# basilevh/occlusions-4d

Hardware: AMD Instinct MI355X
Metric: 4D query-points/sec (encode+decode) at n_points=14336 (higher is better)
Workload: dtype f32; 1 GPU; GREATER inference (BASELINE configs[1]): n_points=14336 video_len=12 num_sample=524288 (-> 534528 grid queries) implicit_batch_size=32768 (decoded in mini-batches of 32256 = 3584 workgroups of 9 queries; every query is decoded, results do not depend on the split), seeded random-init weights; abstract_points=531, outputs_per_query=5, parallelism=single GPU, schedule=sequential, rccl_ranks=1, decode_streams=2, decode_chunk=32256

## Files before the change

occlusions-4d_amd/csrc/pointops.hip:

```cpp
#include "common.hpp"

namespace {

constexpr int TPB = 256;

inline dim3 grid1d(int64_t total) { return dim3((unsigned)((total + TPB - 1) / TPB)); }

__global__ __launch_bounds__(TPB) void pos_hidden_kernel(const float* __restrict__ pos, int64_t ps,
                                                         const float* __restrict__ pos2, int64_t p2s,
                                                         const int32_t* __restrict__ idx, int64_t total, int k, int h,
                                                         const float* __restrict__ P1, const float* __restrict__ c1,
                                                         float* __restrict__ out) {
  const int64_t e = (int64_t)blockIdx.x * TPB + threadIdx.x;
  if (e >= total) return;
  const int m = (int)(e % h);
  const int64_t p = e / h;
  const int64_t i = p / k;
  const int j = idx[p];
  const float* a = pos + i * ps;
  const float* b = pos2 + (int64_t)j * p2s;
  const float dx = a[0] - b[0], dy = a[1] - b[1], dz = a[2] - b[2];
  const float* w = P1 + 3 * m;
  float v = fmaf(dz, w[2], fmaf(dy, w[1], dx * w[0])) + c1[m];
  out[e] = fmaxf(v, 0.f);
}

__global__ __launch_bounds__(TPB) void attn_in_kernel(const float* __restrict__ q, int64_t ldq,
                                                      const float* __restrict__ kf, int64_t ldk,
                                                      const float* __restrict__ pe, const int32_t* __restrict__ idx,
                                                      int64_t total, int k, int d, float* __restrict__ out) {
  const int64_t e = (int64_t)blockIdx.x * TPB + threadIdx.x;
  if (e >= total) return;
  const int c = (int)(e % d);
  const int64_t p = e / d;
  const int64_t i = p / k;
  const int j = idx[p];
  out[e] = (q[i * ldq + c] - kf[(int64_t)j * ldk + c]) + pe[e];
}

template <int KMAX>
__global__ __launch_bounds__(TPB) void softmax_agg_kernel(const float* __restrict__ logits,
                                                          const float* __restrict__ v, int64_t ldv,
                                                          const float* __restrict__ pe,
                                                          const int32_t* __restrict__ idx, int64_t total, int k, int d,
                                                          float divisor, float* __restrict__ agg, int64_t ld_agg) {
  const int64_t e = (int64_t)blockIdx.x * TPB + threadIdx.x;
  if (e >= total) return;
  const int c = (int)(e % d);
  const int64_t i = e / d;
  float a[KMAX];
  float mx = -__builtin_inff();
#pragma unroll
  for (int j = 0; j < KMAX; ++j) {
    if (j < k) {
      a[j] = logits[(i * k + j) * d + c] / divisor;
      mx = fmaxf(mx, a[j]);
    }
  }
  float den = 0.f;
#pragma unroll
  for (int j = 0; j < KMAX; ++j) {
    if (j < k) {
      a[j] = expf(a[j] - mx);
      den += a[j];
    }
  }
  float s = 0.f;
#pragma unroll
  for (int j = 0; j < KMAX; ++j) {
    if (j < k) {
      const int64_t p = i * k + j;
      float val = v[(int64_t)idx[p] * ldv + c];
      if (pe) val += pe[p * d + c];
      s += (a[j] / den) * val;
    }
  }
  agg[i * ld_agg + c] = s;
}

__global__ __launch_bounds__(TPB) void layernorm_kernel(const float* __restrict__ x, int64_t ldx,
                                                        const float* __restrict__ gamma,
                                                        const float* __restrict__ beta, float eps, int relu_out,
                                                        float* __restrict__ y, int64_t ldy, int n, int d) {
  const int row = blockIdx.x * (TPB / 64) + (threadIdx.x >> 6);
  const int lane = threadIdx.x & 63;
  if (row >= n) return;
  const float* xr = x + (int64_t)row * ldx;
  float s = 0.f;
  for (int c = lane; c < d; c += 64) s += xr[c];
#pragma unroll
  for (int o = 32; o > 0; o >>= 1) s += __shfl_xor(s, o);
  const float mean = s / (float)d;
  float q = 0.f;
  for (int c = lane; c < d; c += 64) {
    const float t = xr[c] - mean;
    q += t * t;
  }
#pragma unroll
  for (int o = 32; o > 0; o >>= 1) q += __shfl_xor(q, o);
  const float rstd = 1.0f / sqrtf(q / (float)d + eps);
  float* yr = y + (int64_t)row * ldy;
  for (int c = lane; c < d; c += 64) {
    float t = (xr[c] - mean) * rstd;
    if (gamma) t = t * gamma[c] + beta[c];
    yr[c] = relu_out ? fmaxf(t, 0.f) : t;
  }
}

__global__ __launch_bounds__(TPB) void maxpool_gather_kernel(const float* __restrict__ y, int64_t ldy,
                                                             const int32_t* __restrict__ idx, int64_t total, int k,
                                                             int d, float* __restrict__ z, int64_t ldz) {
  const int64_t e = (int64_t)blockIdx.x * TPB + threadIdx.x;
  if (e >= total) return;
  const int c = (int)(e % d);
  const int64_t i = e / d;
  float m = y[(int64_t)idx[i * k] * ldy + c];
  for (int j = 1; j < k; ++j) m = fmaxf(m, y[(int64_t)idx[i * k + j] * ldy + c]);
  z[i * ldz + c] = m;
}

__global__ __launch_bounds__(TPB) void gather_rows_kernel(const float* __restrict__ src, int64_t lds,
                                                          const int32_t* __restrict__ idx, int64_t total, int d,
                                                          float* __restrict__ out, int64_t ldo) {
  const int64_t e = (int64_t)blockIdx.x * TPB + threadIdx.x;
  if (e >= total) return;
  const int c = (int)(e % d);
  const int64_t i = e / d;
  out[i * ldo + c] = src[(int64_t)idx[i] * lds + c];
}

__global__ __launch_bounds__(TPB) void mean_rows_kernel(const float* __restrict__ x, int64_t ldx, int n, int d,
                                                        float* __restrict__ out) {
  static_assert(TPB == 256, "mean_rows_kernel assumes 256 threads");
  __shared__ float part[8][32];
  const int cl = threadIdx.x & 31, g = threadIdx.x >> 5;
  const int c = blockIdx.x * 32 + cl;
  float s = 0.f;
  if (c < d)
    for (int i = g; i < n; i += 8) s += x[(int64_t)i * ldx + c];
  part[g][cl] = s;
  __syncthreads();
  if (g == 0 && c < d) {
    float t = part[0][cl];
#pragma unroll
    for (int k = 1; k < 8; ++k) t += part[k][cl];
    out[c] = t / (float)n;
  }
}

struct PosencFreqs { float w[16]; };

__global__ __launch_bounds__(TPB) void posenc_kernel(const float* __restrict__ pts, int64_t stride, int64_t total,
                                                     int c, int width, PosencFreqs fr, float* __restrict__ out,
                                                     int64_t ldo) {
  const int64_t e = (int64_t)blockIdx.x * TPB + threadIdx.x;
  if (e >= total) return;
  const int col = (int)(e % width);
  const int64_t i = e / width;
  const float* p = pts + i * stride;
  float v;
  if (col < c) {
    v = p[col];
  } else {
    const int f = (col - c) / (2 * c), r = (col - c) % (2 * c);
    const float arg = p[r % c] * fr.w[f];
    v = r < c ? sinf(arg) : cosf(arg);
  }
  out[i * ldo + col] = v;
}

__global__ __launch_bounds__(TPB) void interp_weights_kernel(const float* __restrict__ dist, int n, int k,
                                                             float* __restrict__ w) {
  const int i = blockIdx.x * TPB + threadIdx.x;
  if (i >= n) return;
  float s = 0.f;
  for (int j = 0; j < k; ++j) {
    const float t = 1.0f / (dist[(int64_t)i * k + j] + 1e-4f);
    w[(int64_t)i * k + j] = t;
    s += fabsf(t);
  }
  s = fmaxf(s, 1e-12f);
  for (int j = 0; j < k; ++j) w[(int64_t)i * k + j] = w[(int64_t)i * k + j] / s;
}

__global__ __launch_bounds__(TPB) void interp_add_kernel(float* __restrict__ x, int64_t ldx,
                                                         const float* __restrict__ cvec,
                                                         const float* __restrict__ table, int64_t ldt,
                                                         const int32_t* __restrict__ idx, const float* __restrict__ w,
                                                         int64_t total, int k, int d) {
  const int64_t e = (int64_t)blockIdx.x * TPB + threadIdx.x;
  if (e >= total) return;
  const int c = (int)(e % d);
  const int64_t i = e / d;
  float s = 0.f;
  for (int j = 0; j < k; ++j) s += w[i * k + j] * table[(int64_t)idx[i * k + j] * ldt + c];
  if (cvec) s += cvec[c];
  x[i * ldx + c] += s;
}

template <int KC>
__global__ __launch_bounds__(TPB) void interp_add4_kernel(float* __restrict__ x, int64_t ldx,
                                                          const float* __restrict__ cvec,
                                                          const float* __restrict__ table, int64_t ldt,
                                                          const int32_t* __restrict__ idx, const float* __restrict__ w,
                                                          int64_t total, int k, int d4) {
  typedef float f4 __attribute__((ext_vector_type(4)));
  const int64_t e = (int64_t)blockIdx.x * TPB + threadIdx.x;
  if (e >= total) return;
  const int c = 4 * (int)(e % d4);
  const int64_t i = e / d4;
  f4 s = {0.f, 0.f, 0.f, 0.f};
  if (KC > 0) {
    int jj[KC > 0 ? KC : 1];
    float wj[KC > 0 ? KC : 1];
    f4 t[KC > 0 ? KC : 1];
#pragma unroll
    for (int j = 0; j < KC; ++j) { jj[j] = idx[i * KC + j]; wj[j] = w[i * KC + j]; }
#pragma unroll
    for (int j = 0; j < KC; ++j) t[j] = *reinterpret_cast<const f4*>(table + (int64_t)jj[j] * ldt + c);
#pragma unroll
    for (int j = 0; j < KC; ++j) { s.x += wj[j] * t[j].x; s.y += wj[j] * t[j].y; s.z += wj[j] * t[j].z; s.w += wj[j] * t[j].w; }
  } else {
    for (int j = 0; j < k; ++j) {
      const float wj = w[i * k + j];
      const f4 t = *reinterpret_cast<const f4*>(table + (int64_t)idx[i * k + j] * ldt + c);
      s.x += wj * t.x; s.y += wj * t.y; s.z += wj * t.z; s.w += wj * t.w;
    }
  }
  if (cvec) {
    const f4 cv = *reinterpret_cast<const f4*>(cvec + c);
    s.x += cv.x; s.y += cv.y; s.z += cv.z; s.w += cv.w;
  }
  f4* xp = reinterpret_cast<f4*>(x + i * ldx + c);
  f4 xv = *xp;
  xv.x += s.x; xv.y += s.y; xv.z += s.z; xv.w += s.w;
  *xp = xv;
}

struct SquashOps { int32_t op[32]; };

__global__ __launch_bounds__(TPB) void squash_kernel(float* __restrict__ out, int64_t ld, int64_t total, int g,
                                                     SquashOps ops) {
  const int64_t e = (int64_t)blockIdx.x * TPB + threadIdx.x;
  if (e >= total) return;
  const int c = (int)(e % g);
  const int64_t i = e / g;
  float v = out[i * ld + c];
  const int op = ops.op[c];
  if (op == 1) v = 1.0f / (1.0f + expf(-v));
  else if (op == 2) v = fminf(fmaxf(v, 0.f), 1.f);
  out[i * ld + c] = v;
}


__global__ __launch_bounds__(256) void matmul_f64_kernel(const double* __restrict__ A, int64_t sam, int64_t sak,
                                                         const double* __restrict__ B, int64_t sbk, int64_t sbn,
                                                         double* __restrict__ Cm, int M, int N, int K) {
  __shared__ double sa[16][17], sb[16][17];
  const int tx = threadIdx.x & 15, ty = threadIdx.x >> 4;
  const int m = blockIdx.y * 16 + ty, n = blockIdx.x * 16 + tx;
  double acc = 0.0;
  for (int k0 = 0; k0 < K; k0 += 16) {
    const int ka = k0 + tx, kb = k0 + ty;
    sa[ty][tx] = (m < M && ka < K) ? A[(int64_t)m * sam + (int64_t)ka * sak] : 0.0;
    sb[ty][tx] = (kb < K && n < N) ? B[(int64_t)kb * sbk + (int64_t)n * sbn] : 0.0;
    __syncthreads();
#pragma unroll
    for (int kk = 0; kk < 16; ++kk) acc = fma(sa[ty][kk], sb[kk][tx], acc);
    __syncthreads();
  }
  if (m < M && n < N) Cm[(int64_t)m * N + n] = acc;
}

}

extern "C" {

int occ4d_pt_pos_hidden_f32(const float* pos, int64_t ps, const float* pos2, int64_t p2s, const int32_t* idx,
                            int n, int k, const float* P1, const float* c1, int h, float* out, void* stream) {
  OCC4D_REQUIRE(pos && pos2 && idx && P1 && c1 && out, "occ4d_pt_pos_hidden_f32: null pointer");
  OCC4D_REQUIRE(n >= 0 && k >= 1 && h >= 1 && ps >= 3 && p2s >= 3, "occ4d_pt_pos_hidden_f32: bad sizes");
  const int64_t total = (int64_t)n * k * h;
  if (!total) return OCC4D_OK;
  pos_hidden_kernel<<<grid1d(total), TPB, 0, (hipStream_t)stream>>>(pos, ps, pos2, p2s, idx, total, k, h, P1, c1, out);
  return occ4d::check_launch("occ4d_pt_pos_hidden_f32");
}

int occ4d_pt_attn_in_f32(const float* q, int64_t ldq, const float* kfeat, int64_t ldk, const float* pe,
                         const int32_t* idx, int n, int k, int d, float* out, void* stream) {
  OCC4D_REQUIRE(q && kfeat && pe && idx && out, "occ4d_pt_attn_in_f32: null pointer");
  OCC4D_REQUIRE(n >= 0 && k >= 1 && d >= 1 && ldq >= d && ldk >= d, "occ4d_pt_attn_in_f32: bad sizes");
  const int64_t total = (int64_t)n * k * d;
  if (!total) return OCC4D_OK;
  attn_in_kernel<<<grid1d(total), TPB, 0, (hipStream_t)stream>>>(q, ldq, kfeat, ldk, pe, idx, total, k, d, out);
  return occ4d::check_launch("occ4d_pt_attn_in_f32");
}

int occ4d_pt_softmax_agg_f32(const float* logits, const float* v, int64_t ldv, const float* pe, const int32_t* idx,
                             int n, int k, int d, float divisor, float* agg, int64_t ld_agg, void* stream) {
  OCC4D_REQUIRE(logits && v && idx && agg, "occ4d_pt_softmax_agg_f32: null pointer");
  OCC4D_REQUIRE(n >= 0 && k >= 1 && k <= 16 && d >= 1 && ldv >= d && ld_agg >= d, "occ4d_pt_softmax_agg_f32: bad sizes");
  OCC4D_REQUIRE(divisor > 0.f, "occ4d_pt_softmax_agg_f32: divisor must be > 0");
  const int64_t total = (int64_t)n * d;
  if (!total) return OCC4D_OK;
  softmax_agg_kernel<16><<<grid1d(total), TPB, 0, (hipStream_t)stream>>>(logits, v, ldv, pe, idx, total, k, d, divisor, agg, ld_agg);
  return occ4d::check_launch("occ4d_pt_softmax_agg_f32");
}

int occ4d_layernorm_f32(const float* x, int64_t ldx, const float* gamma, const float* beta, float eps, int relu_out,
                        float* y, int64_t ldy, int n, int d, void* stream) {
  OCC4D_REQUIRE(x && y, "occ4d_layernorm_f32: null pointer");
  OCC4D_REQUIRE((gamma == nullptr) == (beta == nullptr), "occ4d_layernorm_f32: gamma/beta must both be set or NULL");
  OCC4D_REQUIRE(n >= 0 && d >= 1 && ldx >= d && ldy >= d, "occ4d_layernorm_f32: bad sizes");
  if (!n) return OCC4D_OK;
  layernorm_kernel<<<occ4d::cdiv(n, TPB / 64), TPB, 0, (hipStream_t)stream>>>(x, ldx, gamma, beta, eps, relu_out, y, ldy, n, d);
  return occ4d::check_launch("occ4d_layernorm_f32");
}

int occ4d_maxpool_gather_f32(const float* y, int64_t ldy, const int32_t* idx, int n_out, int k, int d, float* z,
                             int64_t ldz, void* stream) {
  OCC4D_REQUIRE(y && idx && z, "occ4d_maxpool_gather_f32: null pointer");
  OCC4D_REQUIRE(n_out >= 0 && k >= 1 && d >= 1 && ldy >= d && ldz >= d, "occ4d_maxpool_gather_f32: bad sizes");
  const int64_t total = (int64_t)n_out * d;
  if (!total) return OCC4D_OK;
  maxpool_gather_kernel<<<grid1d(total), TPB, 0, (hipStream_t)stream>>>(y, ldy, idx, total, k, d, z, ldz);
  return occ4d::check_launch("occ4d_maxpool_gather_f32");
}

int occ4d_gather_rows_f32(const float* src, int64_t lds, const int32_t* idx, int n_out, int d, float* out,
                          int64_t ldo, void* stream) {
  OCC4D_REQUIRE(src && idx && out, "occ4d_gather_rows_f32: null pointer");
  OCC4D_REQUIRE(n_out >= 0 && d >= 1 && lds >= d && ldo >= d, "occ4d_gather_rows_f32: bad sizes");
  const int64_t total = (int64_t)n_out * d;
  if (!total) return OCC4D_OK;
  gather_rows_kernel<<<grid1d(total), TPB, 0, (hipStream_t)stream>>>(src, lds, idx, total, d, out, ldo);
  return occ4d::check_launch("occ4d_gather_rows_f32");
}

int occ4d_mean_rows_f32(const float* x, int64_t ldx, int n, int d, float* out, void* stream) {
  OCC4D_REQUIRE(x && out, "occ4d_mean_rows_f32: null pointer");
  OCC4D_REQUIRE(n >= 1 && d >= 1 && ldx >= d, "occ4d_mean_rows_f32: bad sizes");
  mean_rows_kernel<<<occ4d::cdiv(d, 32), TPB, 0, (hipStream_t)stream>>>(x, ldx, n, d, out);
  return occ4d::check_launch("occ4d_mean_rows_f32");
}

int occ4d_posenc_f32(const float* pts, int64_t stride, int n, int c, int n_freq, double base_freq, float* out,
                     int64_t ldo, void* stream) {
  OCC4D_REQUIRE(pts && out, "occ4d_posenc_f32: null pointer");
  OCC4D_REQUIRE(n >= 0 && c >= 1 && n_freq >= 0 && n_freq <= 16 && stride >= c, "occ4d_posenc_f32: bad sizes");
  const int width = c * (2 * n_freq + 1);
  OCC4D_REQUIRE(ldo >= width, "occ4d_posenc_f32: ldo too small");
  PosencFreqs fr;
  for (int f = 0; f < 16; ++f) {
    const double omega = base_freq * (double)(1u << f) * 3.141592653589793 * 2.0;
    fr.w[f] = (float)omega;
  }
  const int64_t total = (int64_t)n * width;
  if (!total) return OCC4D_OK;
  posenc_kernel<<<grid1d(total), TPB, 0, (hipStream_t)stream>>>(pts, stride, total, c, width, fr, out, ldo);
  return occ4d::check_launch("occ4d_posenc_f32");
}

int occ4d_interp_weights_f32(const float* dist, int n, int k, float* w, void* stream) {
  OCC4D_REQUIRE(dist && w, "occ4d_interp_weights_f32: null pointer");
  OCC4D_REQUIRE(n >= 0 && k >= 1, "occ4d_interp_weights_f32: bad sizes");
  if (!n) return OCC4D_OK;
  interp_weights_kernel<<<occ4d::cdiv(n, TPB), TPB, 0, (hipStream_t)stream>>>(dist, n, k, w);
  return occ4d::check_launch("occ4d_interp_weights_f32");
}

int occ4d_interp_add_f32(float* x, int64_t ldx, const float* cvec, const float* table, int64_t ldt,
                         const int32_t* idx, const float* w, int n, int k, int d, void* stream) {
  OCC4D_REQUIRE(x && table && idx && w, "occ4d_interp_add_f32: null pointer");
  OCC4D_REQUIRE(n >= 0 && k >= 1 && d >= 1 && ldx >= d && ldt >= d, "occ4d_interp_add_f32: bad sizes");
  const int64_t total = (int64_t)n * d;
  if (!total) return OCC4D_OK;
  const bool vec = d % 4 == 0 && ldx % 4 == 0 && ldt % 4 == 0 && ((uintptr_t)x % 16) == 0 &&
                   ((uintptr_t)table % 16) == 0 && (!cvec || ((uintptr_t)cvec % 16) == 0);
  if (vec) {
    const int64_t total4 = (int64_t)n * (d / 4);
    if (k == 8)
      interp_add4_kernel<8><<<grid1d(total4), TPB, 0, (hipStream_t)stream>>>(x, ldx, cvec, table, ldt, idx, w, total4, k, d / 4);
    else
      interp_add4_kernel<0><<<grid1d(total4), TPB, 0, (hipStream_t)stream>>>(x, ldx, cvec, table, ldt, idx, w, total4, k, d / 4);
  } else {
    interp_add_kernel<<<grid1d(total), TPB, 0, (hipStream_t)stream>>>(x, ldx, cvec, table, ldt, idx, w, total, k, d);
  }
  return occ4d::check_launch("occ4d_interp_add_f32");
}

int occ4d_squash_f32(float* out, int64_t ld, int n, int g, const int32_t* ops_host, void* stream) {
  OCC4D_REQUIRE(out && ops_host, "occ4d_squash_f32: null pointer");
  OCC4D_REQUIRE(n >= 0 && g >= 1 && g <= 32 && ld >= g, "occ4d_squash_f32: need 1 <= g <= 32, ld >= g");
  SquashOps ops;
  for (int i = 0; i < 32; ++i) ops.op[i] = i < g ? ops_host[i] : 0;
  for (int i = 0; i < g; ++i) OCC4D_REQUIRE(ops.op[i] >= 0 && ops.op[i] <= 2, "occ4d_squash_f32: op code %d", ops.op[i]);
  const int64_t total = (int64_t)n * g;
  if (!total) return OCC4D_OK;
  squash_kernel<<<grid1d(total), TPB, 0, (hipStream_t)stream>>>(out, ld, total, g, ops);
  return occ4d::check_launch("occ4d_squash_f32");
}

}

extern "C" int occ4d_matmul_f64(const double* a, int64_t sam, int64_t sak, const double* b, int64_t sbk, int64_t sbn,
                                double* c, int m, int n, int k, void* stream) {
  OCC4D_REQUIRE(a && b && c && m >= 0 && n >= 0 && k >= 1, "occ4d_matmul_f64: bad arguments");
  if (m == 0 || n == 0) return OCC4D_OK;
  matmul_f64_kernel<<<dim3(occ4d::cdiv(n, 16), occ4d::cdiv(m, 16)), 256, 0, (hipStream_t)stream>>>(a, sam, sak, b, sbk,
                                                                                                   sbn, c, m, n, k);
  return occ4d::check_launch("occ4d_matmul_f64");
}
```

profiles/time_interp.py:

```python
import os, sys
import torch
sys.path.insert(0, os.path.dirname(os.path.dirname(os.path.abspath(__file__))))
import occlusions4d_amd as pk
n, m, d, k = 32256, 531, 416, 8
g = torch.Generator(device='cuda').manual_seed(0)
x = torch.randn((n, d), device='cuda', generator=g)
table = torch.randn((m, 6 * d), device='cuda', generator=g)
cv = torch.randn((d,), device='cuda', generator=g)
q = torch.rand((n, 3), device='cuda', generator=g)
a = torch.rand((m, 3), device='cuda', generator=g)
idx, dist = pk.ops.knn(q, a, k, metric=1, return_dist=True)
w = pk.ops.interp_weights(dist)
for _ in range(3):
    pk.ops.interp_add(x, cv, table[:, d:2 * d], idx, w)
torch.cuda.synchronize()
e0, e1 = torch.cuda.Event(enable_timing=True), torch.cuda.Event(enable_timing=True)
e0.record()
for _ in range(50):
    pk.ops.interp_add(x, cv, table[:, d:2 * d], idx, w)
e1.record()
torch.cuda.synchronize()
print('interp_add %.1f us' % (1e3 * e0.elapsed_time(e1) / 50))
```

Before: 4.590 million query-points/s.

## Stage deduplicated interpolation table rows in LDS per 64-row tile

Adds a tiled interp_add kernel for k=8. Each block of 64 query rows builds a shared-memory hash of the distinct neighbour ids. It stages those table rows into LDS once, then computes the weighted sums from LDS instead of re-gathering eight global rows per output vector. It also prefetches x in registers with scheduling barriers. If a tile has too many distinct ids it falls back to a direct gather, and the extra hashing and sync steps add overhead when neighbours barely repeat.

```diff
diff --git a/occlusions-4d_amd/csrc/pointops.hip b/occlusions-4d_amd/csrc/pointops.hip
--- a/occlusions-4d_amd/csrc/pointops.hip
+++ b/occlusions-4d_amd/csrc/pointops.hip
@@ -1,4 +1,6 @@
 #include "common.hpp"
+#include <algorithm>
+#include <cstdlib>
 
 namespace {
 
@@ -237,6 +239,184 @@
   *xp = xv;
 }
 
+constexpr int TILE_R = 64, TILE_NT = 512, TILE_ROWF = 48 * 416, TILE_NIDS = 224;
+constexpr int TILE_MIN_CAP = 32;
+constexpr int TILE_MAX_N = 65536;
+
+template <int R, int NT, int ROWF, int NIDS>
+__global__ __launch_bounds__(NT) __attribute__((amdgpu_waves_per_eu(4, 4)))
+void interp_add_tile_kernel(float* __restrict__ x, int64_t ldx, const float* __restrict__ cvec,
+                            const float* __restrict__ table, int64_t ldt, const int32_t* __restrict__ idx,
+                            const float* __restrict__ w, int n, int d4, int cap) {
+  typedef float f4 __attribute__((ext_vector_type(4)));
+  typedef unsigned u4 __attribute__((ext_vector_type(4)));
+  constexpr int K = 8, NREF = R * K, NSLOT = 2 * NREF, NW = NT / 64;
+  constexpr int XU = 13;
+  constexpr int XA = 4;
+  constexpr int SU = (ROWF / 4 + NT - 1) / NT;
+  static_assert(NREF == NT && (NSLOT & (NSLOT - 1)) == 0, "one reference and two slots per thread");
+  static_assert(NSLOT * 6 <= (ROWF - NREF) * 4 && NIDS <= NREF && NREF <= 65536 && ROWF % 4 == 0,
+                "the hash table fits the row storage in front of the weights");
+  __shared__ __attribute__((aligned(16))) float s_rows[ROWF];
+  __shared__ __attribute__((aligned(16))) unsigned short s_ref[NREF];
+  __shared__ int s_ids[NIDS];
+  __shared__ int s_tot[2 * NW + 1];
+  int* const s_keys = reinterpret_cast<int*>(s_rows);
+  unsigned short* const s_num = reinterpret_cast<unsigned short*>(s_keys + NSLOT);
+  f4* const s_rows4 = reinterpret_cast<f4*>(s_rows);
+  float* const s_w = s_rows + (ROWF - NREF);
+
+  const int tid = threadIdx.x, lane = tid & 63, wave = tid >> 6;
+  const int64_t row0 = (int64_t)blockIdx.x * R;
+  const int rows = (int)(n - row0 < R ? n - row0 : R);
+  const int r_first = tid / d4, c_first = tid - r_first * d4, r_step = NT / d4, c_step = NT - r_step * d4;
+  auto next = [&](int& r, int& c) {
+    r += r_step; c += c_step;
+    if (c >= d4) { c -= d4; ++r; }
+  };
+  char* const xt = reinterpret_cast<char*>(x + row0 * ldx);
+  const unsigned ldxb = (unsigned)ldx * 4u;
+  auto x_at = [&](int r, int c) { return reinterpret_cast<f4*>(xt + ((unsigned)min(r, rows - 1) * ldxb + 16u * (unsigned)c)); };
+  auto sum8 = [&](const f4 wa, const f4 wb, int c, const f4 xin, auto&& t) {
+    const float wj[K] = {wa.x, wa.y, wa.z, wa.w, wb.x, wb.y, wb.z, wb.w};
+    f4 s = {0.f, 0.f, 0.f, 0.f};
+#pragma unroll
+    for (int g = 0; g < K; g += 4) {
+      f4 tj[4];
+#pragma unroll
+      for (int j = 0; j < 4; ++j) tj[j] = t(g + j);
+#pragma unroll
+      for (int j = 0; j < 4; ++j) { s.x += wj[g + j] * tj[j].x; s.y += wj[g + j] * tj[j].y; s.z += wj[g + j] * tj[j].z; s.w += wj[g + j] * tj[j].w; }
+    }
+    if (cvec) {
+      const f4 cv = *reinterpret_cast<const f4*>(cvec + 4 * c);
+      s.x += cv.x; s.y += cv.y; s.z += cv.z; s.w += cv.w;
+    }
+    f4 xo = xin;
+    xo.x += s.x; xo.y += s.y; xo.z += s.z; xo.w += s.w;
+    return xo;
+  };
+
+  f4 xv[XU];
+  int ra = r_first, ca = c_first;
+#pragma unroll
+  for (int u = 0; u < XA; ++u) {
+    xv[u] = *x_at(ra, ca);
+    next(ra, ca);
+  }
+  const bool ref_ok = tid / K < rows;
+  int id = -1;
+  if (ref_ok) {
+    id = idx[row0 * K + tid];
+    s_w[tid] = w[row0 * K + tid];
+  }
+  s_keys[tid] = -1;
+  s_keys[tid + NT] = -1;
+  if (tid == 0) s_tot[2 * NW] = 0;
+  __syncthreads();
+  int slot = 0;
+  if (ref_ok) {
+    if (id < 0) {
+      s_tot[2 * NW] = 1;
+    } else {
+      slot = (int)(((unsigned)id * 2654435761u) >> 16) & (NSLOT - 1);
+      for (int p = 0; p < NSLOT; ++p) {
+        const int old = atomicCAS(&s_keys[slot], -1, id);
+        if (old == -1 || old == id) break;
+        slot = (slot + 1) & (NSLOT - 1);
+      }
+    }
+  }
+  __syncthreads();
+  const int key0 = s_keys[tid], key1 = s_keys[tid + NT];
+  const unsigned long long below = (1ull << lane) - 1ull;
+  const unsigned long long m0 = __ballot(key0 != -1), m1 = __ballot(key1 != -1);
+  if (lane == 0) { s_tot[wave] = __popcll(m0); s_tot[NW + wave] = __popcll(m1); }
+  __syncthreads();
+  int num0 = __popcll(m0 & below), num1 = __popcll(m1 & below), U = 0;
+#pragma unroll
+  for (int q = 0; q < 2 * NW; ++q) {
+    const int t = s_tot[q];
+    if (q < wave) num0 += t;
+    if (q < NW + wave) num1 += t;
+    U += t;
+  }
+  const bool staged = U <= cap && s_tot[2 * NW] == 0;
+  if (key0 != -1) { s_num[tid] = (unsigned short)num0; if (num0 < NIDS) s_ids[num0] = key0; }
+  if (key1 != -1) { s_num[tid + NT] = (unsigned short)num1; if (num1 < NIDS) s_ids[num1] = key1; }
+  __syncthreads();
+  if (ref_ok && id >= 0) s_ref[tid] = s_num[slot];
+  __syncthreads();
+
+  if (!staged) {
+    int* const s_oid = reinterpret_cast<int*>(s_rows);
+    if (ref_ok) s_oid[tid] = id;
+    __syncthreads();
+    auto gathered = [&](int r, int c, const f4 xin) {
+      const u4 ja = *reinterpret_cast<const u4*>(s_oid + r * K), jb = *reinterpret_cast<const u4*>(s_oid + r * K + 4);
+      const int jj[K] = {(int)ja.x, (int)ja.y, (int)ja.z, (int)ja.w, (int)jb.x, (int)jb.y, (int)jb.z, (int)jb.w};
+      return sum8(*reinterpret_cast<const f4*>(s_w + r * K), *reinterpret_cast<const f4*>(s_w + r * K + 4), c, xin,
+                  [&](int j) { return *reinterpret_cast<const f4*>(table + (int64_t)jj[j] * ldt + 4 * c); });
+    };
+    int r = r_first, c = c_first;
+#pragma unroll
+    for (int u = 0; u < XA; ++u) {
+      if (r < rows) *x_at(r, c) = gathered(r, c, xv[u]);
+      next(r, c);
+    }
+    for (; r < rows; next(r, c)) *x_at(r, c) = gathered(r, c, *x_at(r, c));
+    return;
+  }
+
+  f4 tv[SU];
+  {
+    int r = r_first, c = c_first;
+#pragma unroll
+    for (int u = 0; u < SU; ++u) {
+      if (r < U) tv[u] = *reinterpret_cast<const f4*>(table + (int64_t)s_ids[r] * ldt + 4 * c);
+      next(r, c);
+    }
+  }
+  __builtin_amdgcn_sched_barrier(0);
+#pragma unroll
+  for (int u = XA; u < XU; ++u) {
+    xv[u] = *x_at(ra, ca);
+    next(ra, ca);
+  }
+  __builtin_amdgcn_sched_barrier(0);
+  {
+    int r = r_first, c = c_first;
+#pragma unroll
+    for (int u = 0; u < SU; ++u) {
+      if (r < U) s_rows4[tid + u * NT] = tv[u];
+      next(r, c);
+    }
+  }
+  __syncthreads();
+
+  int r = r_first, c = c_first;
+  for (int chunk = 0; r < rows; ++chunk) {
+    if (chunk > 0) {
+#pragma unroll
+      for (int u = 0; u < XU; ++u) {
+        xv[u] = *x_at(ra, ca);
+        next(ra, ca);
+      }
+    }
+#pragma unroll
+    for (int u = 0; u < XU; ++u) {
+      const int rr = min(r, rows - 1);
+      const u4 p = *reinterpret_cast<const u4*>(s_ref + rr * K);
+      const unsigned pj[K] = {p.x & 0xffffu, p.x >> 16, p.y & 0xffffu, p.y >> 16, p.z & 0xffffu, p.z >> 16, p.w & 0xffffu, p.w >> 16};
+      const f4 xo = sum8(*reinterpret_cast<const f4*>(s_w + rr * K), *reinterpret_cast<const f4*>(s_w + rr * K + 4), c, xv[u],
+                         [&](int j) { return s_rows4[pj[j] * d4 + c]; });
+      if (r < rows) *x_at(r, c) = xo;
+      next(r, c);
+      __builtin_amdgcn_sched_barrier(0);
+    }
+  }
+}
+
 struct SquashOps { int32_t op[32]; };
 
 __global__ __launch_bounds__(TPB) void squash_kernel(float* __restrict__ out, int64_t ld, int64_t total, int g,
@@ -377,7 +557,14 @@
   if (!total) return OCC4D_OK;
   const bool vec = d % 4 == 0 && ldx % 4 == 0 && ldt % 4 == 0 && ((uintptr_t)x % 16) == 0 &&
                    ((uintptr_t)table % 16) == 0 && (!cvec || ((uintptr_t)cvec % 16) == 0);
-  if (vec) {
+  static const bool tile_on = [] { const char* e = getenv("OCC4D_INTERP_TILE"); return !(e && e[0] == '0' && !e[1]); }();
+  const bool tile = vec && k == 8 && tile_on && d <= (TILE_ROWF - 8 * TILE_R) / TILE_MIN_CAP && ldx <= (1 << 22) &&
+                    n <= TILE_MAX_N;
+  if (tile) {
+    const int cap = std::min((TILE_ROWF - 8 * TILE_R) / d, TILE_NIDS);
+    interp_add_tile_kernel<TILE_R, TILE_NT, TILE_ROWF, TILE_NIDS><<<occ4d::cdiv(n, TILE_R), TILE_NT, 0, (hipStream_t)stream>>>(
+        x, ldx, cvec, table, ldt, idx, w, n, d / 4, cap);
+  } else if (vec) {
     const int64_t total4 = (int64_t)n * (d / 4);
     if (k == 8)
       interp_add4_kernel<8><<<grid1d(total4), TPB, 0, (hipStream_t)stream>>>(x, ldx, cvec, table, ldt, idx, w, total4, k, d / 4);
diff --git a/profiles/time_interp.py b/profiles/time_interp.py
--- a/profiles/time_interp.py
+++ b/profiles/time_interp.py
@@ -3,21 +3,50 @@
 sys.path.insert(0, os.path.dirname(os.path.dirname(os.path.abspath(__file__))))
 import occlusions4d_amd as pk
 n, m, d, k = 32256, 531, 416, 8
+dev = torch.device('cuda:0')
 g = torch.Generator(device='cuda').manual_seed(0)
-x = torch.randn((n, d), device='cuda', generator=g)
-table = torch.randn((m, 6 * d), device='cuda', generator=g)
-cv = torch.randn((d,), device='cuda', generator=g)
-q = torch.rand((n, 3), device='cuda', generator=g)
-a = torch.rand((m, 3), device='cuda', generator=g)
-idx, dist = pk.ops.knn(q, a, k, metric=1, return_dist=True)
-w = pk.ops.interp_weights(dist)
-for _ in range(3):
-    pk.ops.interp_add(x, cv, table[:, d:2 * d], idx, w)
-torch.cuda.synchronize()
-e0, e1 = torch.cuda.Event(enable_timing=True), torch.cuda.Event(enable_timing=True)
-e0.record()
-for _ in range(50):
-    pk.ops.interp_add(x, cv, table[:, d:2 * d], idx, w)
-e1.record()
-torch.cuda.synchronize()
-print('interp_add %.1f us' % (1e3 * e0.elapsed_time(e1) / 50))
+
+
+def bench_lists():
+    pa, ia, inf = pk.configs.model_args('greater', 14336)
+    esd, _ = pk.configs.synthetic_weights(pa, ia, 0)
+    enc = pk.model.PointCompletionNetV3(**pa).to(dev).eval()
+    enc.load_state_dict(esd)
+    with torch.no_grad():
+        abstract = enc(pk.configs.synthetic_pcl('greater', 14336, 12, 0).to(dev), False)[0].squeeze(0)
+    grid = pk.geometry.sample_implicit_points_blind_device(524288, inf['min_z'], inf['cube_bounds'], 3, inf['data_kind'],
+                                                           inf['cube_mode'], 'grid', dev)
+    b = (grid.shape[0] // 2) // n * n
+    idx, dist = pk.ops.knn(grid[b:b + n], abstract[:, :3].contiguous(), k, metric=1, return_dist=True)
+    return idx, pk.ops.interp_weights(dist), abstract.shape[0]
+
+
+def time_case(name, idx, w, rows, n_rows=n):
+    x = torch.randn((n_rows, d), device='cuda', generator=g)
+    table = torch.randn((rows, 6 * d), device='cuda', generator=g)
+    cv = torch.randn((d,), device='cuda', generator=g)
+    for _ in range(3):
+        pk.ops.interp_add(x, cv, table[:, d:2 * d], idx, w)
+    torch.cuda.synchronize()
+    best = []
+    for _ in range(3):
+        e0, e1 = torch.cuda.Event(enable_timing=True), torch.cuda.Event(enable_timing=True)
+        e0.record()
+        for _ in range(50):
+            pk.ops.interp_add(x, cv, table[:, d:2 * d], idx, w)
+        e1.record()
+        torch.cuda.synchronize()
+        best.append(1e3 * e0.elapsed_time(e1) / 50)
+    print('interp_add %-46s %s us' % (name, '  '.join('%.1f' % t for t in best)), flush=True)
+
+
+idx, w, m_abs = bench_lists()
+time_case('(a) bench lists (%d x %d, %d table rows)' % (n, d, m_abs), idx, w, m_abs)
+idx = torch.randint(0, m, (n, k), device='cuda', generator=g, dtype=torch.int32)
+w = torch.rand((n, k), device='cuda', generator=g)
+time_case('(b) random lists over %d rows' % m, idx, w, m)
+time_case('(c) k = 1 (streaming floor)', idx[:, :1].contiguous(), w[:, :1].contiguous(), m)
+n_train = 68812
+idx = torch.randint(0, m, (n_train, k), device='cuda', generator=g, dtype=torch.int32)
+w = torch.rand((n_train, k), device='cuda', generator=g)
+time_case('(d) random lists, %d x %d' % (n_train, d), idx, w, m, n_train)
```

Result: no change. 4.618 million query-points/s (median of 6 runs) (+0.6%).
